# titoeb/RecModel

Hardware: AMD Instinct MI355X
Metric: ALS user+item row-updates/sec (higher is better)
Workload: dtype f32; 1 GPU; cfg3: WMF k=128+bias, 10000000x1000000 CSR, 99990947 nnz, alpha-log confidence, gamma=0.1, zipf_a=0.0; n_items=1000000, nnz=99990947, k=128, bias=True

## Files before the change

include/wmf_hip.h:

```cpp
#ifndef WMF_HIP_H
#define WMF_HIP_H

#include <stdint.h>

#ifdef __cplusplus
extern "C" {
#endif

#define WMF_OK            0
#define WMF_EINVAL       -1
#define WMF_EHIP         -2
#define WMF_ENOMEM       -3
#define WMF_ENUMERIC     -4

#define WMF_MAX_F        260

typedef struct wmf_plan wmf_plan;

const char* wmf_last_error(void);
int  wmf_version(void);
int  wmf_ld_for(int f);

int wmf_recompute_factors_host(const float* Y_host, int64_t m, int f, int bias,
                               const int64_t* indptr, const int32_t* indices, const float* values,
                               int64_t n, double lambda, float* X_host);

int64_t wmf_gram_workspace_bytes(int f);

int wmf_gram(const float* Y, int64_t m, int f, int ld, int bias,
             double* G_sum, void* workspace, void* stream);

int wmf_factorize(const double* G_sum, int f, int ld, double lambda,
                  float* W_white, float* W_unwhite, int32_t* info,
                  void* workspace, void* stream);

int wmf_rolled_layout_supported(int f, int ld);

int wmf_row_transform(const float* in, int64_t m, int f, int ld, const float* W,
                      int set_col0_one, float* out, float* col0_out, void* stream);
int wmf_whitened_row_floats(int f, int ld, int bias);

int wmf_chained_supported(int f, int ld, int bias);
int wmf_gram_whitened(const float* g, int64_t m, int f, int ld, int bias,
                      double* G_aug, void* workspace, void* stream);
int wmf_compose_whitening(const double* G_aug, const float* U, int f, int ld, int bias, int rolled, double lambda,
                          float* W_white, float* W_unwhite, float* N_ext, int32_t* info,
                          void* workspace, void* stream);
int wmf_row_transform_chained(const float* g, int64_t m, int f, int ld, int bias, const float* N_ext, int rolled,
                              float* out, float* col0_out, void* stream);

int  wmf_plan_create(const int64_t* indptr_host, int64_t n, int f, int bias, wmf_plan** out);
void wmf_plan_destroy(wmf_plan* p);
int  wmf_plan_stats(const wmf_plan* p, int64_t* out14);
int  wmf_plan_iter_stats(wmf_plan* p, int64_t* out4);

int wmf_solve_rows(const wmf_plan* plan, const float* V, const float* bias_fixed,
                   const int64_t* indptr, const int32_t* indices, const float* values,
                   int64_t n, int f, int ld, float* g, int32_t* fail_count, void* stream);
#define WMF_SOLVE_ROLLED 1
int wmf_solve_rows_ex(const wmf_plan* plan, const float* V, const float* bias_fixed,
                   const int64_t* indptr, const int32_t* indices, const float* values,
                   int64_t n, int f, int ld, float* g, int32_t* fail_count, int flags, void* stream);

int64_t wmf_eval_workspace_bytes(void);
int wmf_eval_sqerr(const float* users, const float* items, int f, int ld, int bias,
                   const int64_t* indptr, const int32_t* indices, const float* values,
                   int64_t n, double* out3, void* workspace, void* stream);

int64_t wmf_audit_workspace_bytes(int64_t n);
int wmf_half_step_audit(const float* X, const float* Y, int f, int ld, int bias,
                        const int64_t* indptr, const int32_t* indices, const float* values, int64_t n,
                        const double* dense, double* out_sums, double* out_rows,
                        void* workspace, int64_t workspace_bytes, void* stream);
int wmf_half_step_audit_f64(const double* X, const double* Y, int f, int bias,
                            const int64_t* indptr, const int32_t* indices, const double* values, int64_t n,
                            const double* dense, double* out_sums, double* out_rows,
                            void* workspace, int64_t workspace_bytes, void* stream);

#define WMF_EXPLAIN_MAX_TARGETS 16
int64_t wmf_explain_workspace_bytes(int64_t n, int f, int32_t n_targets);
int wmf_explain_rows(const float* Y, int64_t m, int f, int ld, int bias, const float* W_white,
                     const int64_t* indptr, const int32_t* indices, const float* values, int64_t n,
                     const int32_t* targets, int32_t n_targets,
                     float* out_contrib, float* out_total, int32_t* fail_count,
                     void* workspace, int64_t workspace_bytes, void* stream);

int64_t wmf_foldin_workspace_bytes(int64_t n, int f);
int wmf_foldin_rows(const float* Y, int64_t m, int f, int ld, int bias, const float* W_white,
                    const int64_t* indptr, const int32_t* indices, const float* values, int64_t n,
                    float* X_out, int32_t* fail_count,
                    void* workspace, int64_t workspace_bytes, void* stream);

int wmf_predict_pairs(const float* users, const float* items, int f, int ld, int bias,
                      const int32_t* users_idx, int64_t n_u, const int32_t* items_idx, int64_t n_i,
                      float* out, void* stream);

int64_t wmf_rank_workspace_bytes(int64_t n_cand);
// ... 178 lines not shown
```

recmodel_amd/_lib.py:

```python
import ctypes
import os

import torch

_HERE = os.path.dirname(os.path.abspath(__file__))
LIB_PATH = os.environ.get("WMF_HIP_LIB", os.path.join(_HERE, "libwmf_hip.so"))

WMF_OK, WMF_EINVAL, WMF_EHIP, WMF_ENOMEM, WMF_ENUMERIC = 0, -1, -2, -3, -4

c_int, c_i64, c_dbl, c_vp = ctypes.c_int, ctypes.c_int64, ctypes.c_double, ctypes.c_void_p

SIGNATURES = {
    "wmf_last_error": (ctypes.c_char_p, []),
    "wmf_version": (c_int, []),
    "wmf_ld_for": (c_int, [c_int]),
    "wmf_recompute_factors_host": (c_int, [c_vp, c_i64, c_int, c_int, c_vp, c_vp, c_vp, c_i64, c_dbl, c_vp]),
    "wmf_gram_workspace_bytes": (c_i64, [c_int]),
    "wmf_gram": (c_int, [c_vp, c_i64, c_int, c_int, c_int, c_vp, c_vp, c_vp]),
    "wmf_factorize": (c_int, [c_vp, c_int, c_int, c_dbl, c_vp, c_vp, c_vp, c_vp, c_vp]),
    "wmf_row_transform": (c_int, [c_vp, c_i64, c_int, c_int, c_vp, c_int, c_vp, c_vp, c_vp]),
    "wmf_whitened_row_floats": (c_int, [c_int, c_int, c_int]),
    "wmf_chained_supported": (c_int, [c_int, c_int, c_int]),
    "wmf_gram_whitened": (c_int, [c_vp, c_i64, c_int, c_int, c_int, c_vp, c_vp, c_vp]),
    "wmf_compose_whitening": (c_int, [c_vp, c_vp, c_int, c_int, c_int, c_int, c_dbl, c_vp, c_vp, c_vp, c_vp, c_vp, c_vp]),
# ... 42 lines not shown
                                 c_vp, c_vp, c_vp, c_vp, c_i64, c_vp]),
    "wmf_rerank_mmr_resident_pool": (c_i64, [c_int, c_int]),
    "wmf_rerank_mmr": (c_int, [c_vp, c_i64, c_int, c_int, c_int, c_vp, c_vp, c_vp, c_vp, c_i64, c_i64, ctypes.c_float, c_i64, c_vp, c_vp,
                               c_vp, c_vp, c_vp]),
    "wmf_intra_list_similarity": (c_int, [c_vp, c_i64, c_int, c_int, c_int, c_vp, c_vp, c_vp, c_i64, c_i64, c_vp, c_vp, c_vp]),
    "wmf_rank_positions_workspace_bytes": (c_i64, [c_i64, c_i64, c_int]),
    "wmf_rank_positions": (c_int, [c_vp, c_vp, c_int, c_int, c_int, c_vp, c_i64, c_i64, c_vp, c_vp, c_vp, c_vp, c_int, c_vp, c_vp,
                                   c_vp, c_i64, c_vp]),
    "wmf_hit_counts": (c_int, [c_vp, c_vp, c_int, c_int, c_int, c_vp, c_vp, c_vp, c_i64, c_vp, c_int, c_vp, c_vp, c_int, c_vp, c_vp]),
    "wmf_spmm_rows": (c_int, [c_vp, c_vp, c_vp, c_vp, c_i64, c_int, c_int, c_vp, c_vp]),
    "wmf_gather_rows": (c_int, [c_vp, c_int, c_vp, c_i64, c_vp, c_vp]),
    "wmf_coo_to_csr_workspace_bytes": (c_i64, [c_i64, c_i64, c_i64]),
    "wmf_coo_to_csr": (c_int, [c_vp, c_vp, c_vp, c_i64, c_i64, c_i64, c_vp, c_vp, c_vp, c_vp, c_vp, c_i64, c_vp]),
    "wmf_confidence_transform": (c_int, [c_vp, c_i64, c_dbl, c_dbl, c_int, c_vp]),
    "wmf_confidence_transform_f64": (c_int, [c_vp, c_i64, c_dbl, c_dbl, c_int, c_vp]),
    "wmf_half_step_f64_workspace_bytes": (c_i64, [c_int, c_i64, c_i64]),
    "wmf_half_step_f64": (c_int, [c_vp, c_i64, c_int, c_int, c_vp, c_vp, c_vp, c_i64, c_dbl, c_vp, c_vp, c_i64, c_vp, c_vp]),
    "wmf_recompute_factors_f64_host": (c_int, [c_vp, c_i64, c_int, c_int, c_vp, c_vp, c_vp, c_i64, c_dbl, c_vp]),
    "wmf_profile_enable": (c_int, [c_int]),
    "wmf_profile_set_tag": (c_int, [c_int]),
    "wmf_profile_collect": (c_int, []),
    "wmf_profile_entry": (c_int, [c_int, c_vp, c_int, c_vp, c_vp, c_vp, c_vp, c_vp]),
    "wmf_profile_reset": (c_int, []),
    "wmf_debug_set_flags": (c_int, [c_int]),
    "wmf_debug_get_flags": (c_int, []),
}

DEBUG_FLAGS = {
    "WMF_DBG_NO_ELIMINATION": 1,
    "WMF_DBG_NO_ACCUMULATION": 2,
    "WMF_DBG_NO_TILE_INVERSE": 8,
    "WMF_DBG_LOW32_GAUSS_JORDAN": 64,
    "WMF_DBG_NO_BORDER": 256,
    "WMF_DBG_WIDE_EIGHT_WAVES": 1024,
    "WMF_DBG_NO_ROW_PAIRS": 2048,
    "WMF_DBG_HEAVY_REG_RING": 4096,
    "WMF_DBG_HEAVY_F32_ACC": 8192,
    "WMF_DBG_HEAVY_REG_RING_K64": 65536,
    "WMF_DBG_F32_GRAM": 131072,
    "WMF_DBG_F32_TRANSFORM": 262144,
    "WMF_DBG_LOW_F32_TILES": 524288,
    "WMF_DBG_WIDE_F32": 2097152,
    "WMF_DBG_HEAVY_ONE_WAVE": 16777216,
    "WMF_DBG_HEAVY_PIVOTED_LU": 33554432,
    "WMF_DBG_F64_TEAMS": 67108864,
    "WMF_DBG_F64_NO_LOW_RANK": 134217728,
    "WMF_DBG_NO_ITER": 268435456,
    "WMF_DBG_F64_VALU": 536870912,
    "WMF_DBG_NO_ROLLED_LAYOUT": 1073741824,
}
SHIPPED_DEBUG_FLAGS = ("WMF_DBG_HEAVY_REG_RING", "WMF_DBG_F32_GRAM", "WMF_DBG_HEAVY_ONE_WAVE", "WMF_DBG_F64_NO_LOW_RANK",
                       "WMF_DBG_NO_ITER", "WMF_DBG_F64_VALU")


def parse_debug_flags(text):
    value = 0
    for part in str(text).split("|"):
        part = part.strip()
        name = part if part.startswith("WMF_DBG_") else "WMF_DBG_" + part
        value |= DEBUG_FLAGS[name] if name in DEBUG_FLAGS else int(part, 0)
    return value


class WmfLibraryError(RuntimeError):
    """libwmf_hip.so is missing or a HIP call failed."""


class WmfNumericError(ArithmeticError):
    """The Gramian was not positive definite or a row system was singular."""


_lib = None


def load():
    global _lib
    if _lib is not None:
        return _lib
    if not os.path.exists(LIB_PATH):
        raise WmfLibraryError(
            f"{LIB_PATH} is not built; run `python -c 'import __graft_entry__ as g; g.build()'` "
            "or `make -C recmodel_amd/csrc`.  There is no CPU fallback for the WMF hot path.")
    lib = ctypes.CDLL(LIB_PATH)
    for name, (res, args) in SIGNATURES.items():
        fn = getattr(lib, name)
        fn.restype, fn.argtypes = res, args
    flags = os.environ.get("WMF_DEBUG_FLAGS")
    if flags and lib.wmf_debug_set_flags(parse_debug_flags(flags)) != WMF_OK:
        raise ValueError(lib.wmf_last_error().decode("utf-8", "replace"))
    _lib = lib
    return lib


def profile_table(lib=None):
    lib = lib or load()
    out = []
    name = ctypes.create_string_buffer(200)
    tag, n = c_int(), c_i64()
    ms, lo, hi = c_dbl(), c_dbl(), c_dbl()
    for i in range(lib.wmf_profile_collect()):
        check(lib.wmf_profile_entry(i, name, 200, ctypes.byref(tag), ctypes.byref(ms), ctypes.byref(n), ctypes.byref(lo),
                                    ctypes.byref(hi)))
        out.append((name.value.decode(), tag.value, ms.value, n.value, lo.value, hi.value))
    return out


# ... 17 lines not shown
```

recmodel_amd/csrc/wmf_api.hip:

```cpp
#include "../../include/wmf_hip.h"
#include "wmf_internal.h"

#include <atomic>
#include <cstdarg>
#include <cstdio>
#include <cstring>
#include <mutex>
#include <set>
#include <string>
#include <vector>

static thread_local char g_err[512] = "";
int wmf_debug_flags = 0;

void wmf_set_error(const char* fmt, ...) {
    va_list ap;
    va_start(ap, fmt);
    vsnprintf(g_err, sizeof(g_err), fmt, ap);
    va_end(ap);
}

#define HIP_TRY(call)                                                                            \
    do {                                                                                         \
        hipError_t e_ = (call);                                                                  \
// ... 222 lines not shown
    double* gA = (double*)((char*)workspace + gram_a_off(f));
    wmf_launch_factorize(G_sum, f, ld, lambda, W_white, W_unwhite, info, gA, (hipStream_t)stream);
    return check_launch("wmf_factorize");
}

int wmf_row_transform(const float* in, int64_t m, int f, int ld, const float* W, int set_col0_one, float* out,
                      float* col0_out, void* stream) {
    int rc = check_shape(f, ld);
    if (rc) return rc;
    if (!in || !W || !out || m < 0) { wmf_set_error("wmf_row_transform: null pointer or negative m"); return WMF_EINVAL; }
    rc = wmf_launch_transform(in, m, f, ld, W, set_col0_one, out, col0_out, (hipStream_t)stream);
    if (rc) {
        if (rc == WMF_L_LAYOUT) wmf_set_error("wmf_row_transform: f=%d, ld=%d with set_col0_one writes the split layout: col0_out (float[2 m]) is required and out may not alias in", f, ld);
        else wmf_set_error("wmf_row_transform: unsupported f=%d", f);
        return WMF_EINVAL;
    }
    return check_launch("wmf_row_transform");
}

int wmf_chained_supported(int f, int ld, int bias) {
    if (check_shape(f, ld)) return 0;
    const int f1 = f + (bias ? 1 : 0);
    return (f >= 97 && f1 <= 144 && ld >= f1 && f + 1 <= WMF_MAX_F) ? 1 : 0;
}
static int check_chained(const char* what, int f, int ld, int bias) {
    if (wmf_chained_supported(f, ld, bias)) return WMF_OK;
    wmf_set_error("%s: unsupported f=%d, ld=%d, bias=%d (wmf_chained_supported)", what, f, ld, bias);
    return WMF_EINVAL;
}

int wmf_gram_whitened(const float* g, int64_t m, int f, int ld, int bias, double* G_aug, void* workspace, void* stream) {
    if (check_chained("wmf_gram_whitened", f, ld, bias)) return WMF_EINVAL;
    if (!g || !G_aug || !workspace || m < 0) { wmf_set_error("wmf_gram_whitened: null pointer or negative m"); return WMF_EINVAL; }
    {
        const int f1 = f + (bias ? 1 : 0);
        const int64_t nfb = (f1 + 15) / 16, nt = nfb * (nfb + 1) / 2;
        if ((int64_t)wmf_gram_nwaves(m, f1) * nt * 256 * (int64_t)sizeof(float) > gram_partial_bytes(f + 1)) {
            wmf_set_error("wmf_gram_whitened: workspace layout too small at f=%d", f);
            return WMF_EINVAL;
        }
    }
    if (wmf_launch_gram_aug(g, m, f, ld, bias, G_aug, (float*)workspace, (double*)((char*)workspace + gram_slices_off(f + 1)),
                            (hipStream_t)stream)) {
        wmf_set_error("wmf_gram_whitened: unsupported f=%d", f);
        return WMF_EINVAL;
    }
    return check_launch("wmf_gram_whitened");
}

int wmf_compose_whitening(const double* G_aug, const float* U, int f, int ld, int bias, int rolled, double lambda, float* W_white,
                          float* W_unwhite, float* N_ext, int32_t* info, void* workspace, void* stream) {
    if (check_chained("wmf_compose_whitening", f, ld, bias)) return WMF_EINVAL;
    if (!G_aug || !U || !W_white || !W_unwhite || !N_ext || !info || !workspace) { wmf_set_error("wmf_compose_whitening: null pointer"); return WMF_EINVAL; }
    if (rolled && !(bias && wmf_rolled_layout(f, ld))) { wmf_set_error("wmf_compose_whitening: rolled needs wmf_rolled_layout_supported(f=%d, ld=%d) and bias", f, ld); return WMF_EINVAL; }
    if (U == W_unwhite || U == W_white) { wmf_set_error("wmf_compose_whitening: U may not alias an output"); return WMF_EINVAL; }
    wmf_launch_compose(G_aug, U, f, ld, bias, rolled, lambda, W_white, W_unwhite, N_ext, info, (double*)workspace,
                       (double*)((char*)workspace + gram_a_off(f + 1)), (hipStream_t)stream);
    return check_launch("wmf_compose_whitening");
}

int wmf_row_transform_chained(const float* g, int64_t m, int f, int ld, int bias, const float* N_ext, int rolled, float* out,
                              float* col0_out, void* stream) {
    if (check_chained("wmf_row_transform_chained", f, ld, bias)) return WMF_EINVAL;
    if (!g || !N_ext || !out || m < 0) { wmf_set_error("wmf_row_transform_chained: null pointer or negative m"); return WMF_EINVAL; }
    const int rc = wmf_launch_transform_chained(g, m, f, ld, bias, N_ext, rolled, out, col0_out, (hipStream_t)stream);
    if (rc) {
        if (rc == WMF_L_LAYOUT) wmf_set_error("wmf_row_transform_chained: f=%d, ld=%d: col0_out is required with biases and out may not alias g in the split layout", f, ld);
        else wmf_set_error("wmf_row_transform_chained: unsupported f=%d, ld=%d, rolled=%d", f, ld, rolled);
        return WMF_EINVAL;
    }
    return check_launch("wmf_row_transform_chained");
}

static int bin_of(int64_t d, int f) {
    if (d <= 16) return WMF_BIN_LOW16;
    if (d <= 32) return WMF_BIN_LOW32;
    return wmf_direct_supported(f) ? WMF_BIN_MFMA : WMF_BIN_GENERAL;
}

int wmf_plan_create(const int64_t* indptr, int64_t n, int f, int bias, wmf_plan** out) {
    if (!indptr || !out || n < 0 || n > 0x7fffffffLL) { wmf_set_error("wmf_plan_create: bad arguments"); return WMF_EINVAL; }
    if (f < 1 || f > WMF_MAX_F) { wmf_set_error("wmf_plan_create: f=%d unsupported", f); return WMF_EINVAL; }
    wmf_plan* p = new wmf_plan();
    memset(p, 0, sizeof(*p));
    p->n = n; p->f = f;
    std::vector<int32_t> order((size_t)n);
    int64_t start[WMF_NBINS + 1] = {0};
    for (int64_t r = 0; r < n; ++r) {
        const int64_t d = indptr[r + 1] - indptr[r];
        if (d < 0) { delete p; wmf_set_error("wmf_plan_create: indptr not monotone at row %lld", (long long)r); return WMF_EINVAL; }
        p->count[bin_of(d, f)]++;
        p->nnz[bin_of(d, f)] += d;
    }
    for (int b = 0; b < WMF_NBINS; ++b) start[b + 1] = start[b] + p->count[b];
    int64_t fill[WMF_NBINS];
    for (int b = 0; b < WMF_NBINS; ++b) fill[b] = start[b];
    const int hb = wmf_direct_supported(f) ? WMF_BIN_MFMA : WMF_BIN_GENERAL;
    const bool can_split = wmf_direct_supported(f) || wmf_rowsplit_supported(f);
    std::vector<int32_t> heavy;
    for (int64_t r = 0; r < n; ++r) {
        const int64_t d = indptr[r + 1] - indptr[r];
        if (d <= 8) { order[(size_t)fill[WMF_BIN_LOW16]++] = (int32_t)r; p->count8++; p->nnz8 += d; }
    }
    const bool split_layout = bias && wmf_split_layout(f, wmf_ld_for(f));
    const int64_t iter_dmax = wmf_iter_dmax(f, wmf_ld_for(f), split_layout ? 1 : 0);
    p->iter_dmax = (int)iter_dmax;
    std::vector<int32_t> longer;
// ... 694 lines not shown
```

recmodel_amd/csrc/wmf_dense.hip:

```cpp
#include "wmf_common.h"
#include "wmf_internal.h"

#include <type_traits>
#include <utility>

template <int NFB, int NSPLIT, int S>
__device__ __forceinline__ void gram_body(const float* __restrict__ Y, int64_t m, int f, int ld, int bias,
                                          float* __restrict__ partial, int64_t step_lo, int64_t step_hi) {
    constexpr int NT = NFB * (NFB + 1) / 2;
    constexpr int NACC = (NT + NSPLIT - 1) / NSPLIT;
    const int lane = threadIdx.x & 63;
    const int r = lane & 15, q = lane >> 4;
    f32x4 acc[NACC];
#pragma unroll
    for (int i = 0; i < NACC; ++i) acc[i] = f32x4{0.f, 0.f, 0.f, 0.f};

    constexpr int U = 4;
    float cur[U][NFB], nxt[U][NFB];
    const int last_col = min(16 * (NFB - 1) + r, ld - 1);
    const float col_mask_last = (16 * (NFB - 1) + r < f) ? 1.f : 0.f;
    auto load_trip = [&](int64_t s0, float (&fr)[U][NFB]) {
#pragma unroll
        for (int uu = 0; uu < U; ++uu) {
            const int64_t row = min(4 * (s0 + uu) + q, m - 1);
// ... 342 lines not shown
        const int j = lane;
        double v = (i == j) ? 1.0 : 0.0;
        const double gv = G[min(i, f - 1) * f + min(j, f - 1)];
        if (i < f && j < f) v = gv + (i == j ? lambda : 0.0);
        Gs[i * FZ_LD + j] = v;
        Xs[i * FZ_LD + j] = 0.0;
    }
    __builtin_amdgcn_fence(__ATOMIC_RELEASE, "wavefront");
    __builtin_amdgcn_wave_barrier();
    int fail = 0;
    auto tile = [&](double* M, int bi, int bj) { return M + (16 * bi) * FZ_LD + 16 * bj; };
    auto sync = [&]() { __builtin_amdgcn_fence(__ATOMIC_RELEASE, "wavefront"); __builtin_amdgcn_wave_barrier(); };
    for (int p = 0; p < nb; ++p) {
        const int bad = fz_diag(tile(Gs, p, p), tile(Gs, p, p), tile(Xs, p, p), FZ_LD, lane);
        if (bad && !fail) fail = 16 * p + bad;
        sync();
        for (int i = p + 1; i < nb; ++i) {
            const f64x4 c = fz_mul_abt(tile(Gs, i, p), FZ_LD, tile(Xs, p, p), FZ_LD, f64x4{0.0, 0.0, 0.0, 0.0}, r, q, 1.0);
            sync();
            fz_store(tile(Gs, i, p), FZ_LD, c, r, q);
            sync();
        }
        for (int i = p + 1; i < nb; ++i)
            for (int j = p + 1; j <= i; ++j) {
                const f64x4 c = fz_mul_abt(tile(Gs, i, p), FZ_LD, tile(Gs, j, p), FZ_LD, fz_load(tile(Gs, i, j), FZ_LD, r, q), r, q, -1.0);
                fz_store(tile(Gs, i, j), FZ_LD, c, r, q);
            }
        sync();
    }
    for (int p = 0; p < nb; ++p)
        for (int i = p + 1; i < nb; ++i) {
            f64x4 sacc = f64x4{0.0, 0.0, 0.0, 0.0};
            for (int k = p; k < i; ++k) sacc = fz_mul_ab(tile(Gs, i, k), FZ_LD, tile(Xs, k, p), FZ_LD, sacc, r, q, 1.0);
            fz_store(Ts, FZ_LD, sacc, r, q);
            sync();
            const f64x4 c = fz_mul_ab(tile(Xs, i, i), FZ_LD, Ts, FZ_LD, f64x4{0.0, 0.0, 0.0, 0.0}, r, q, -1.0);
            fz_store(tile(Xs, i, p), FZ_LD, c, r, q);
            sync();
        }
    const bool ok = fail == 0;
    if (lane == 0 && !ok) *info = fail;
#pragma unroll 8
    for (int i = 0; i < 64; ++i) {
        if (i >= f) break;
        for (int j = lane; j < ld; j += 64) {
            float wu = 0.f, ww = 0.f;
            if (j < f && ok) { wu = (float)Xs[i * FZ_LD + j]; ww = (float)Xs[j * FZ_LD + i]; }
            Wunwhite[i * ld + j] = wu;
            Wwhite[i * ld + j] = ww;
        }
    }
}

__global__ __launch_bounds__(512, 1) void factorize_blocked_kernel(const double* __restrict__ G, int f, int ld, double lambda,
                                                                   float* __restrict__ Wwhite, float* __restrict__ Wunwhite,
                                                                   int32_t* __restrict__ info, double* __restrict__ work) {
    __shared__ __attribute__((aligned(16))) double Ts[8][16 * 18];
    __shared__ int bad;
    const int tid = threadIdx.x, lane = tid & 63, r = lane & 15, q = lane >> 4;
    const int wave = __builtin_amdgcn_readfirstlane(tid >> 6);
    const int nb = (f + 15) >> 4, fp = 16 * nb, LD = fp + 2;
    double* A = work;
    double* X = work + (size_t)fp * LD;
    if (tid == 0) bad = 0;
    for (int e = tid; e < fp * fp; e += 512) {
        const int i = e / fp, j = e % fp;
        double v = (i == j) ? 1.0 : 0.0;
        if (i < f && j < f) v = G[i * f + j] + (i == j ? lambda : 0.0);
        A[i * LD + j] = v;
        X[i * LD + j] = 0.0;
    }
    __syncthreads();
    auto tile = [&](double* M, int bi, int bj) { return M + (size_t)(16 * bi) * LD + 16 * bj; };
    for (int p = 0; p < nb; ++p) {
        if (wave == 0) {
            const int fail = fz_diag(tile(A, p, p), tile(A, p, p), tile(X, p, p), LD, lane);
            if (fail && lane == 0 && !bad) bad = 16 * p + fail;
        }
        __syncthreads();
        for (int i = p + 1 + wave; i < nb; i += 8) {
            const f64x4 c = fz_mul_abt(tile(A, i, p), LD, tile(X, p, p), LD, f64x4{0.0, 0.0, 0.0, 0.0}, r, q, 1.0);
            fz_store(tile(A, i, p), LD, c, r, q);
        }
        __syncthreads();
        int t = 0;
        for (int i = p + 1; i < nb; ++i)
            for (int j = p + 1; j <= i; ++j, ++t) {
                if ((t & 7) != wave) continue;
                const f64x4 c = fz_mul_abt(tile(A, i, p), LD, tile(A, j, p), LD, fz_load(tile(A, i, j), LD, r, q), r, q, -1.0);
                fz_store(tile(A, i, j), LD, c, r, q);
            }
        __syncthreads();
    }
    double* ts = Ts[wave];
    for (int p = wave; p < nb; p += 8)
        for (int i = p + 1; i < nb; ++i) {
            f64x4 sacc = f64x4{0.0, 0.0, 0.0, 0.0};
            for (int k = p; k < i; ++k) sacc = fz_mul_ab(tile(A, i, k), LD, tile(X, k, p), LD, sacc, r, q, 1.0);
            fz_store(ts, 18, sacc, r, q);
            __builtin_amdgcn_fence(__ATOMIC_RELEASE, "wavefront");
            __builtin_amdgcn_wave_barrier();
            const f64x4 c = fz_mul_ab(tile(X, i, i), LD, ts, 18, f64x4{0.0, 0.0, 0.0, 0.0}, r, q, -1.0);
            fz_store(tile(X, i, p), LD, c, r, q);
            __builtin_amdgcn_fence(__ATOMIC_RELEASE, "wavefront");
            __builtin_amdgcn_wave_barrier();
        }
    __syncthreads();
    const bool ok = bad == 0;
    if (tid == 0 && !ok) *info = bad;
    for (int e = tid; e < f * ld; e += 512) {
        const int i = e / ld, j = e % ld;
        float wu = 0.f, ww = 0.f;
        if (j < f && ok) { wu = (float)X[i * LD + j]; ww = (float)X[j * LD + i]; }
        Wunwhite[e] = wu;
        Wwhite[e] = ww;
    }
}

int wmf_launch_factorize(const double* G_sum, int f, int ld, double lambda, float* Wwhite, float* Wunwhite,
                         int32_t* info, double* gA, hipStream_t st) {
    if (f <= 64) {
        WmfProfScope ps("factorize64m_kernel", st);
        hipLaunchKernelGGL(factorize64m_kernel, dim3(1), dim3(64), 0, st, G_sum, f, ld, lambda, Wwhite, Wunwhite, info);
        return 0;
    }
    WmfProfScope ps("factorize_blocked_kernel", st);
    hipLaunchKernelGGL(factorize_blocked_kernel, dim3(1), dim3(512), 0, st, G_sum, f, ld, lambda, Wwhite, Wunwhite, info, gA);
    return 0;
}

template <int NFB, bool W_IN_LDS, int NB0 = 0, int NBW = NFB>
__global__ __launch_bounds__(512) void transform_kernel(const float* __restrict__ in, int64_t m, int f, int ld,
                                                        const float* __restrict__ W, int set_col0_one,
                                                        float* __restrict__ out, float* __restrict__ col0_out,
                                                        int64_t nblocks16) {
    extern __shared__ __attribute__((aligned(16))) char smem_raw[];
    float* Wl = reinterpret_cast<float*>(smem_raw);
    constexpr int KP = 16 * NFB;
    constexpr int NP = 16 * NBW;
    constexpr int LDW = NP + 4;
    const int tid = threadIdx.x;
    __shared__ int nz[NFB * NBW];
    for (int e = tid; e < NFB * NBW; e += 512) nz[e] = 0;
    __syncthreads();
    for (int e = tid; e < KP * LDW; e += 512) {
        const int a = e / LDW, b = e % LDW, col = 16 * NB0 + b;
        const float v = (a < f && b < NP && col < f) ? W[a * ld + col] : 0.f;
        if constexpr (W_IN_LDS) Wl[e] = v;
        if (v != 0.f) nz[(a >> 4) * NBW + (b >> 4)] = 1;
    }
    __syncthreads();
    const int lane = tid & 63, wv = tid >> 6;
    const int r = lane & 15, q = lane >> 4;
    const int nch = ld >> 2;
    unsigned tmask[NFB];
#pragma unroll
    for (int t = 0; t < NFB; ++t) {
        unsigned mk = 0;
#pragma unroll
        for (int nb = 0; nb < NBW; ++nb) mk |= nz[t * NBW + nb] ? (1u << nb) : 0u;
        tmask[t] = __builtin_amdgcn_readfirstlane(mk);
    }
    constexpr bool DBL = NFB <= 11;
    const int64_t stride = (int64_t)gridDim.x * 8;
    auto request = [&](int64_t blk, float4 (&x)[NFB]) {
        const int64_t row = blk * 16 + r;
        const float4* irow = reinterpret_cast<const float4*>(in + (row < m ? row : 0) * (int64_t)ld);
#pragma unroll
        for (int t = 0; t < NFB; ++t) x[t] = irow[min(4 * t + q, nch - 1)];
    };
    auto block = [&](int64_t blk, float4 (&xc)[NFB], float4 (&xn)[NFB]) {
        if constexpr (DBL) { if (blk + stride < nblocks16) request(blk + stride, xn); }
        const int64_t row = blk * 16 + r;
        const bool rok = row < m;
        f32x4 acc[NBW];
#pragma unroll
        for (int nb = 0; nb < NBW; ++nb) acc[nb] = f32x4{0.f, 0.f, 0.f, 0.f};
#pragma unroll
        for (int t = 0; t < NFB; ++t) {
            const int c = 4 * t + q;
// ... 263 lines not shown
            launch_transform_slice<NFB, H, NFB - H>(in, m, f, ld, W, set_col0_one, out, col0_out, grid, nblk, st);
        } else {
            launch_transform_slice<NFB, 0, 6>(in, m, f, ld, W, set_col0_one, out, col0_out, grid, nblk, st);
            launch_transform_slice<NFB, 6, 6>(in, m, f, ld, W, set_col0_one, out, col0_out, grid, nblk, st);
            launch_transform_slice<NFB, 12, NFB - 12>(in, m, f, ld, W, set_col0_one, out, col0_out, grid, nblk, st);
        }
    } else {
        static const char* nm = wmf_kname("transform_kernel<%d, false, 0, %d>", NFB, NFB);
        WMF_LAUNCH(nm, (transform_kernel<NFB, false>), dim3((unsigned)grid), dim3(512), 0, st, in, m, f, ld, W,
                   set_col0_one, out, col0_out, nblk);
    }
    return WMF_L_OK;
}

int wmf_launch_transform(const float* in, int64_t m, int f, int ld, const float* W, int set_col0_one, float* out,
                         float* col0_out, hipStream_t st) {
    if (m <= 0) return WMF_L_OK;
    const int nfb = (f + 15) / 16;
    if (set_col0_one == 3 || set_col0_one == 4) {
        if (!wmf_rolled_layout(f, ld)) return WMF_L_NO_KERNEL;
    } else {
        set_col0_one = set_col0_one ? (wmf_split_layout(f, ld) ? 2 : 1) : 0;
    }
    if ((set_col0_one == 2 || set_col0_one == 3) && (!col0_out || in == out)) return WMF_L_LAYOUT;
    return wmf_dispatch_nfb<1, 17>(nfb, [&](auto n) { return launch_transform_nfb<decltype(n)::value>(in, m, f, ld, W, set_col0_one, out, col0_out, st); });
}

__device__ __forceinline__ double compose_t(const float* __restrict__ U, int f, int ld, int bias, int rolled, int p, int j) {
    if (p >= f) return j == 0 ? 1.0 : 0.0;
    if (bias && j == 0) return 0.0;
    const int src = rolled ? (p + 1 == f ? 0 : p + 1) : p;
    return (double)U[src * ld + j];
}
template <class FA, class FB>
__device__ __forceinline__ double compose_dot16(int n, FA a, FB b) {
    double s = 0.0;
#pragma unroll 3
    for (int k = threadIdx.x & 15; k < n; k += 16) s += a(k) * b(k);
#pragma unroll
    for (int off = 8; off; off >>= 1) s += __shfl_xor(s, off, 16);
    return s;
}
__global__ __launch_bounds__(256) void compose_h_kernel(const double* __restrict__ Gaug, const float* __restrict__ U, int f, int ld,
                                                        int bias, int rolled, double* __restrict__ H) {
    const int f1 = f + (bias ? 1 : 0);
    const int e0 = (blockIdx.x * blockDim.x + threadIdx.x) >> 4;
    const bool live = e0 < f1 * f;
    const int e = live ? e0 : 0;
    const int p = e / f, j = e - p * f;
    const double s = compose_dot16(f1, [&](int k) { return Gaug[p * f1 + k]; }, [&](int k) { return compose_t(U, f, ld, bias, rolled, k, j); });
    if (live && (threadIdx.x & 15) == 0) H[e] = s;
}
__global__ __launch_bounds__(256) void compose_g_kernel(const double* __restrict__ H, const float* __restrict__ U, int f, int ld,
                                                        int bias, int rolled, double* __restrict__ Gt) {
    const int f1 = f + (bias ? 1 : 0);
    const int e0 = (blockIdx.x * blockDim.x + threadIdx.x) >> 4;
    const bool live = e0 < f * f;
    const int e = live ? e0 : 0;
    int i = e / f, j = e - i * f;
    if (i > j) { const int t = i; i = j; j = t; }
    const double s = compose_dot16(f1, [&](int p) { return compose_t(U, f, ld, bias, rolled, p, i); }, [&](int p) { return H[p * f + j]; });
    if (live && (threadIdx.x & 15) == 0) Gt[e] = s;
}
__global__ __launch_bounds__(256) void compose_n_kernel(const float* __restrict__ U, const float* __restrict__ Ww, int f, int ld,
                                                        int bias, int rolled, float* __restrict__ N) {
    const int f1 = f + (bias ? 1 : 0);
    const int e0 = (blockIdx.x * blockDim.x + threadIdx.x) >> 4;
    const bool live = e0 < f1 * ld;
    const int e = live ? e0 : 0;
    const int p = e / ld, n = e - p * ld;
    const int col = n >= f ? 0 : rolled ? (n + 1 == f ? 0 : n + 1) : n;
    double s = compose_dot16(f, [&](int j) { return compose_t(U, f, ld, bias, rolled, p, j); }, [&](int j) { return (double)Ww[j * ld + col]; });
    if (n >= f) s = (n == f && bias && p < f) ? (double)U[(rolled ? (p + 1 == f ? 0 : p + 1) : p) * ld] : 0.0;
    if (live && (threadIdx.x & 15) == 0) N[e] = (float)s;
}

int wmf_launch_compose(const double* G_aug, const float* U, int f, int ld, int bias, int rolled, double lambda, float* Wwhite,
                       float* Wunwhite, float* N_ext, int32_t* info, double* scratch, double* gA, hipStream_t st) {
    const int f1 = f + (bias ? 1 : 0);
    double* H = scratch;
    double* Gt = scratch + (size_t)f1 * f;
    WMF_LAUNCH("compose_h_kernel", compose_h_kernel, dim3((f1 * f + 15) / 16), dim3(256), 0, st, G_aug, U, f, ld, bias, rolled, H);
    WMF_LAUNCH("compose_g_kernel", compose_g_kernel, dim3((f * f + 15) / 16), dim3(256), 0, st, H, U, f, ld, bias, rolled, Gt);
    wmf_launch_factorize(Gt, f, ld, lambda, Wwhite, Wunwhite, info, gA, st);
    WMF_LAUNCH("compose_n_kernel", compose_n_kernel, dim3((f1 * ld + 15) / 16), dim3(256), 0, st, U, Wwhite, f, ld, bias, rolled, N_ext);
    return WMF_L_OK;
}

template <int NFB, int MODE>
__global__ __launch_bounds__(512) void chain6_kernel(const float* __restrict__ in, int64_t m, int f, int ld,
                                                     const float* __restrict__ W,
                                                     float* __restrict__ out, float* __restrict__ col0_out,
                                                     int64_t nblocks16) {
    extern __shared__ __attribute__((aligned(16))) char smem_raw[];
    constexpr int NP = 16 * NFB;
    constexpr int NKC = (NP + 31) / 32;
    constexpr int KS = 176;
    static_assert(32 * NKC <= KS, "K does not fit the LDS row");
    __bf16* Wt = reinterpret_cast<__bf16*>(smem_raw);
    __shared__ int nz[NKC * NFB];
    const int tid = threadIdx.x;
    constexpr bool bias = MODE != 0;
    const int f1 = f + (bias ? 1 : 0);
    for (int e = tid; e < NKC * NFB; e += 512) nz[e] = 0;
    __syncthreads();
    typedef __bf16 stage_bf16x8 __attribute__((ext_vector_type(8)));
    stage_bf16x8* Ws = reinterpret_cast<stage_bf16x8*>(Wt);
    for (int it = tid; it < NP * (KS / 8); it += 512) {
        const int k8 = it / NP, n = it - k8 * NP;
        float v[8];
#pragma unroll
        for (int j = 0; j < 8; ++j) {
            const int k = 8 * k8 + j;
            const bool in_w = k < f1 && n < f1;
            v[j] = W[in_w ? k * ld + n : 0];
            if (!in_w) v[j] = 0.f;
        }
        stage_bf16x8 ph, pm, pl;
        bool any = false;
#pragma unroll
        for (int j = 0; j < 8; ++j) {
            const __bf16 h = (__bf16)v[j];
            const float r1 = v[j] - (float)h;
            const __bf16 md = (__bf16)r1;
            ph[j] = h; pm[j] = md; pl[j] = (__bf16)(r1 - (float)md);
            any |= v[j] != 0.f;
        }
        const int at = (n * KS + 8 * k8) / 8;
        Ws[at] = ph;
        Ws[NP * KS / 8 + at] = pm;
        Ws[2 * NP * KS / 8 + at] = pl;
        if (any) nz[(k8 >> 2) * NFB + (n >> 4)] = 1;
    }
    __syncthreads();
    const int lane = tid & 63, wv = __builtin_amdgcn_readfirstlane(tid >> 6);
    const int r = lane & 15, q = lane >> 4;
    const int nch = ld >> 2;
    unsigned cmask[NKC];
#pragma unroll
    for (int c = 0; c < NKC; ++c) {
        unsigned mk = 0;
#pragma unroll
        for (int nb = 0; nb < NFB; ++nb) mk |= nz[c * NFB + nb] ? (1u << nb) : 0u;
        cmask[c] = __builtin_amdgcn_readfirstlane(mk);
    }
    typedef __bf16 bf16x8_t __attribute__((ext_vector_type(8)));
    const bf16x8_t* Wl = reinterpret_cast<const bf16x8_t*>(Wt);
    const int64_t stride = (int64_t)gridDim.x * 8;
    auto request = [&](int64_t blk, float4 (&x)[2 * NKC]) {
        const int64_t row = blk * 16 + r;
        const float4* irow = reinterpret_cast<const float4*>(in + (row < m ? row : 0) * (int64_t)ld);
#pragma unroll
        for (int c = 0; c < NKC; ++c) {
            x[2 * c] = irow[min(8 * c + 2 * q, nch - 1)];
            x[2 * c + 1] = irow[min(8 * c + 2 * q + 1, nch - 1)];
        }
    };
    constexpr bool sp = MODE == 2 || MODE == 3;
    const int fcol = f & 15;
    auto block = [&](int64_t blk, float4 (&xc)[2 * NKC]) {
        f32x4 acc[NFB];
#pragma unroll
        for (int nb = 0; nb < NFB; ++nb) acc[nb] = f32x4{0.f, 0.f, 0.f, 0.f};
#pragma unroll
        for (int c = 0; c < NKC; ++c) {
            const int k0 = 32 * c + 8 * q;
            float xe[8] = {xc[2 * c].x, xc[2 * c].y, xc[2 * c].z, xc[2 * c].w, xc[2 * c + 1].x, xc[2 * c + 1].y, xc[2 * c + 1].z, xc[2 * c + 1].w};
            if (32 * c + 32 > 16 * (NFB - 1)) {
#pragma unroll
                for (int e = 0; e < 8; ++e) if (!(k0 + e < f)) xe[e] = (bias && k0 + e == f) ? 1.f : 0.f;
            }
            bf16x8_t ah, am, al;
#pragma unroll
            for (int e = 0; e < 8; ++e) {
                const __bf16 h = (__bf16)xe[e];
                const float r1 = xe[e] - (float)h;
                const __bf16 md = (__bf16)r1;
                ah[e] = h; am[e] = md; al[e] = (__bf16)(r1 - (float)md);
            }
            unsigned mv = cmask[c];
            asm volatile("" : "+v"(mv));
            const unsigned mk = __builtin_amdgcn_readfirstlane(mv);
#pragma unroll
            for (int nb = 0; nb < NFB; ++nb) {
                if (!(mk & (1u << nb))) continue;
                const int at = ((16 * nb + r) * KS + 32 * c + 8 * q) / 8;
                const bf16x8_t bh = Wl[at], bm = Wl[NP * KS / 8 + at], bl = Wl[2 * NP * KS / 8 + at];
                f32x4 cc = acc[nb];
                cc = __builtin_amdgcn_mfma_f32_16x16x32_bf16(al, bh, cc, 0, 0, 0);
                cc = __builtin_amdgcn_mfma_f32_16x16x32_bf16(am, bm, cc, 0, 0, 0);
                cc = __builtin_amdgcn_mfma_f32_16x16x32_bf16(ah, bl, cc, 0, 0, 0);
                cc = __builtin_amdgcn_mfma_f32_16x16x32_bf16(am, bh, cc, 0, 0, 0);
                cc = __builtin_amdgcn_mfma_f32_16x16x32_bf16(ah, bm, cc, 0, 0, 0);
                cc = __builtin_amdgcn_mfma_f32_16x16x32_bf16(ah, bh, cc, 0, 0, 0);
                acc[nb] = cc;
            }
        }
        const int wid = sp ? f - 1 : ld;
        const bool stuff = MODE == 3 && (r & 7) < 2;
        const int stuff_sh = 2 * (r >> 3) + (r & 7);
        auto store_rows = [&](auto full) {
#pragma unroll
            for (int reg = 0; reg < 4; ++reg) {
                const int64_t orow = blk * 16 + 4 * q + reg;
                const float bias_src = acc[NFB - 1][reg];
                const unsigned bbits = MODE == 3 ? (unsigned)__builtin_amdgcn_ds_bpermute((16 * q + fcol) * 4, __builtin_bit_cast(int, bias_src)) : 0u;
                if (decltype(full)::value || orow < m) {
                    float* o = out + orow * (int64_t)wid;
#pragma unroll
                    for (int nb = 0; nb < NFB; ++nb) {
                        const int col = 16 * nb + r;
                        float v = acc[nb][reg];
                        if (MODE == 3 && 16 * nb < 128) {
                            const unsigned vb = __builtin_bit_cast(unsigned, v);
                            v = __builtin_bit_cast(float, stuff ? ((vb & ~1u) | ((bbits >> (4 * nb + stuff_sh)) & 1u)) : vb);
                        }
                        if (nb < NFB - 1) { o[col] = v; continue; }
                        if (col < wid) o[col] = col < f ? v : 0.f;
// ... 42 lines not shown
```

recmodel_amd/csrc/wmf_internal.h:

```cpp
#pragma once
#include <hip/hip_runtime.h>
#include <stdint.h>
#include <type_traits>
#include <utility>
#include "../../include/wmf_hip.h"
#include "wmf_filter.h"

#define WMF_GRAM_MAX_WAVES 4096
#define WMF_EVAL_MAX_BLOCKS 2048
#define WMF_AUDIT_MAX_BLOCKS 2048
#define WMF_HEAVY_T 4096
#define WMF_SEG 2048
#define WMF_WIDE_LU_GRID 64

extern int wmf_debug_flags;
#ifdef WMF_LAB
constexpr bool WMF_LAB_BUILD = true;
#else
constexpr bool WMF_LAB_BUILD = false;
#endif
constexpr int WMF_DBG_SHIPPED = WMF_DBG_HEAVY_REG_RING | WMF_DBG_F32_GRAM | WMF_DBG_HEAVY_ONE_WAVE | WMF_DBG_F64_NO_LOW_RANK |
                                WMF_DBG_NO_ITER | WMF_DBG_F64_VALU;
constexpr int WMF_DBG_LAB = WMF_DBG_NO_ELIMINATION | WMF_DBG_NO_ACCUMULATION | WMF_DBG_NO_TILE_INVERSE | WMF_DBG_LOW32_GAUSS_JORDAN |
                            WMF_DBG_NO_BORDER | WMF_DBG_WIDE_EIGHT_WAVES | WMF_DBG_NO_ROW_PAIRS | WMF_DBG_HEAVY_F32_ACC |
                            WMF_DBG_HEAVY_REG_RING_K64 | WMF_DBG_F32_TRANSFORM | WMF_DBG_LOW_F32_TILES | WMF_DBG_WIDE_F32 |
                            WMF_DBG_HEAVY_PIVOTED_LU | WMF_DBG_F64_TEAMS | WMF_DBG_NO_ROLLED_LAYOUT;
constexpr int WMF_DBG_ACCEPTED = WMF_LAB_BUILD ? (WMF_DBG_SHIPPED | WMF_DBG_LAB) : WMF_DBG_SHIPPED;

enum { WMF_BIN_LOW16 = 0, WMF_BIN_LOW32 = 1, WMF_BIN_MFMA = 2, WMF_BIN_GENERAL = 3, WMF_NBINS = 4 };

struct wmf_plan {
    int64_t n;
    int f;
    int64_t count[WMF_NBINS];
    int64_t count8, nnz8;
    bool bias;
    bool split;
    int64_t nnz[WMF_NBINS];
    int32_t* rows[WMF_NBINS];
    int32_t* rows_all;
    int32_t* fallback_rows;
    int32_t* fallback_count;
    float* w_eff;
    int64_t heavy_count, heavy_nnz, seg_total;
    int64_t* seg_lo;
    int32_t* seg_d;
    int32_t* seg_first;
    float* partial;
    float* wide_ws;
    int64_t iter_count, iter_nnz;
    int iter_dmax;
    int32_t* iter_bounce_rows;
    int32_t* iter_info;
    unsigned long long* iter_stats;
};

int wmf_gram_max_waves(int f);
int wmf_gram_nwaves(int64_t m, int f);
int wmf_launch_gram(const float* Y, int64_t m, int f, int ld, int bias, double* G_sum, float* partial, double* slices,
                    hipStream_t st);
int wmf_launch_factorize(const double* G_sum, int f, int ld, double lambda, float* Wwhite, float* Wunwhite,
                         int32_t* info, double* gA, hipStream_t st);
int wmf_launch_transform(const float* in, int64_t m, int f, int ld, const float* W, int set_col0_one, float* out,
                         float* col0_out, hipStream_t st);
int wmf_launch_gram_aug(const float* g, int64_t m, int f, int ld, int bias, double* G_aug, float* partial, double* slices,
                        hipStream_t st);
int wmf_launch_compose(const double* G_aug, const float* U, int f, int ld, int bias, int rolled, double lambda, float* Wwhite,
                       float* Wunwhite, float* N_ext, int32_t* info, double* scratch, double* gA, hipStream_t st);
int wmf_launch_transform_chained(const float* g, int64_t m, int f, int ld, int bias, const float* N_ext, int rolled, float* out,
                                 float* col0_out, hipStream_t st);

enum WmfLaunchRc { WMF_L_OK = 0, WMF_L_NO_KERNEL = -1, WMF_L_HIP = -2, WMF_L_LAYOUT = -3, WMF_L_TOO_MANY_KEYS = -4 };

struct RowArgs {
    const float* V; const float* side; const float* biasv; int bstride;
    const int64_t* indptr; const int32_t* indices; const float* vals;
    int f, ld; float* g; int32_t* fb_rows; int32_t* fb_count; int32_t* fail_count;
    int dbg; bool rolled; hipStream_t st;
};
struct RowList { const int32_t* rows; int64_t count; const int32_t* count_dev; };

template <int N>
using wmf_int = std::integral_constant<int, N>;
template <int... NS, class Fn>
static inline int wmf_dispatch_list(int n, Fn&& fn) {
    int rc = WMF_L_NO_KERNEL;
    (void)(... || (n == NS ? ((rc = fn(wmf_int<NS>{})), true) : false));
    return rc;
}
template <int LO, class Fn, int... IS>
static inline int wmf_dispatch_seq(int n, Fn&& fn, std::integer_sequence<int, IS...>) { return wmf_dispatch_list<(LO + IS)...>(n, fn); }
template <int LO, int HI, class Fn>
static inline int wmf_dispatch_nfb(int n, Fn&& fn) { return wmf_dispatch_seq<LO>(n, fn, std::make_integer_sequence<int, HI - LO + 1>{}); }
template <class Fn>
static inline int wmf_dispatch_dw(int f, bool border, Fn&& fn) {
    if (border) return wmf_dispatch_list<1, 2, 4, 5, 6, 8>(f / 16, [&](auto n) { return fn(n, std::true_type{}); });
    return wmf_dispatch_nfb<1, 9>((f + 15) / 16, [&](auto n) { return fn(n, std::false_type{}); });
}

int wmf_launch_solve(const wmf_plan* plan, const RowArgs& a);
static inline int wmf_direct_supported(int f) { return f >= 1 && f <= 144; }
static inline bool wmf_dw_border(int f) { return f > 16 && f <= 144 && f % 16 == 1 && (f / 16) % 4 != 3 && !(wmf_debug_flags & WMF_DBG_NO_BORDER); }
static inline bool wmf_split_layout(int f, int ld) { return wmf_dw_border(f) && ld == f + 3; }
int wmf_directl_supported(int f, int ld);
int wmf_launch_directl(const RowArgs& a, RowList l);
int wmf_launch_directl_segments(const wmf_plan* pl, const RowArgs& a);
int wmf_launch_directw(const wmf_plan* pl, const RowArgs& a);
int64_t wmf_directw_partial_floats(int f);
int wmf_launch_accumulate(const RowArgs& a, const int32_t* degrees, int64_t n, float* partial, int slot_stride, int slot_offset);
int wmf_launch_eliminate(const RowArgs& a, float* partial, int64_t n, int slots_per_row);
void wmf_launch_bias_adjust(const float* vals, const int32_t* indices, const float* biasv, int64_t nnz, float* w_eff,
                            hipStream_t st);
int64_t wmf_csr_ws_bytes(int64_t nnz, int64_t n_rows, int64_t n_cols);
int wmf_launch_coo_to_csr(const int64_t* rows, const int64_t* cols, const float* vals, int64_t nnz, int64_t n_rows, int64_t n_cols,
                          int64_t* indptr, int32_t* indices, float* values, int32_t* bad_flag, void* ws, hipStream_t st);
int wmf_wide_supported(int f);
int wmf_launch_wide(const RowArgs& a, RowList l);
int wmf_iter_dmax(int f, int ld, int split);
int wmf_launch_iter(const wmf_plan* pl, const RowArgs& a, RowList l);
static inline bool wmf_iter_enabled() { return !(wmf_debug_flags & WMF_DBG_NO_ITER); }
// ... 139 lines not shown
```

recmodel_amd/engine.py:

```python
import ctypes
import os

import numpy as np
import torch

from . import _lib


def _ptr(t):
    return ctypes.c_void_p(t.data_ptr()) if t is not None else None


def _stream():
    return ctypes.c_void_p(torch.cuda.current_stream().cuda_stream)


class _HeldWork:

    def __init__(self, work, *buffers, landing=None):
        self.work, self.buffers, self.landing = work, buffers, landing

    def wait(self):
        self.work.wait()
        if self.landing is not None:
# ... 707 lines not shown
    def _publish(self, side, c, force=False):
        if not self.exchange:
            return
        if self.reduce[self._other(side)] and not force:
            self._stale[side] = True
            return
        lo, ln = self.chunk_bounds[side][c]
        W = self.world
        if self.sparse[side]:
            need = self.need[side]
            start, stop = self.chunk_range[side][c]
            rows = need["send_idx"][c]
            send = self.K.gather_rows(self.factors[side], rows) if hasattr(self.K, "gather_rows") else self.factors[side].index_select(0, rows)
            self._pending[side].append(self._all_to_all_rows(self.X[side][start:stop], send, need["recv_counts"][c],
                                                             need["send_counts"][c]))
            return
        self._pending[side].append(torch.distributed.all_gather_into_tensor(
            self.X[side][W * lo: W * (lo + ln)], self.factors[side][lo: lo + ln], group=self.group, async_op=True))

    def _all_to_all_rows(self, out, send, recv_counts, send_counts):
        if torch.distributed.get_backend(self.group) == "nccl" or not out.is_cuda:
            work = torch.distributed.all_to_all_single(out, send, list(recv_counts), list(send_counts), group=self.group, async_op=True)
            return _HeldWork(work, send)
        torch.cuda.current_stream().synchronize()
        send_h, out_h = send.cpu(), torch.empty(out.shape, dtype=out.dtype)
        work = torch.distributed.all_to_all_single(out_h, send_h, list(recv_counts), list(send_counts), group=self.group, async_op=True)
        return _HeldWork(work, send_h, landing=(out, out_h))

    def _ensure_gathered(self, side):
        if self._stale[side]:
            self._stale[side] = False
            for c in range(len(self.chunk_bounds[side])):
                self._publish(side, c, force=True)
        self._wait(side)

    def _wait(self, side):
        for work in self._pending[side]:
            if work is not None:
                work.wait()
        self._pending[side] = []

    def _invalidate(self, side):
        self.g_valid[side] = self._owed[side] = False

    def _materialize(self, side):
        if self._owed[side]:
            self._owed[side] = False
            self.K.row_transform(self.g[side], self.n_local[side], self.f, self.ld, self.U[side], self.unwhite_mode,
                                 self.factors.raw(side), None)

    def _prepare_chained(self, fixed):
        K, n = self.K, self.n_local[fixed]
        K.gram_whitened(self.g[fixed], n, self.f, self.ld, self.bias, self.G_aug, self.ws)
        K.compose_whitening(self.G_aug, self.U[fixed], self.f, self.ld, self.bias, self.rolled, self.gamma, self.W_white,
                            self.W_unwhite, self.N_ext, self.info, self.ws)
        K.row_transform_chained(self.g[fixed], n, self.f, self.ld, self.bias, self.N_ext, self.rolled, self.V[fixed],
                                self.bias_vec[fixed] if self.bias else None)

    def prepare(self, fixed):
        K = self.K
        self._fixed_from_g = self.chained and self.g_valid[fixed]
        if self._fixed_from_g:
            return self._prepare_chained(fixed)
        blk = self.factors[fixed]
        K.gram(blk, self.n_local[fixed], self.f, self.ld, self.bias, self.G, self.ws)
        if self.exchange:
            torch.distributed.all_reduce(self.G, group=self.group)
        K.factorize(self.G, self.f, self.ld, self.gamma, self.W_white, self.W_unwhite, self.info, self.ws)
        V, bvec = self.V[fixed], self.bias_vec[fixed]
        if not self.exchange:
            K.row_transform(self.X[fixed], self.n_local[fixed], self.f, self.ld, self.W_white, self.white_mode, V,
                            bvec if self.bias else None)
            return
        if self._stale[fixed]:
            self._ensure_gathered(fixed)
        pending, self._pending[fixed] = self._pending[fixed], []
        done = len(self.chunk_bounds[fixed]) - len(pending)
        for c, (start, stop) in enumerate(self.chunk_range[fixed]):
            if c >= done and pending[c - done] is not None:
                pending[c - done].wait()
            rows = slice(start, stop)
            if stop > start:
                K.row_transform(self.X[fixed][rows], stop - start, self.f, self.ld, self.W_white, self.white_mode, V[rows],
                                bvec[rows] if self.bias else None)

    def update(self, side):
        K = self.K
        fixed = self._other(side)
        bvec = self.bias_vec[fixed] if self.bias else None
        self._wait(side)
        self._invalidate(side)
        for c, ((lo, ln), csr) in enumerate(zip(self.chunk_bounds[side], self.csr_chunks[side])):
            g = self.g[side][lo: lo + ln]
            K.solve_rows(csr._plan, self.V[fixed], bvec, csr.indptr, csr.indices, csr.values, ln, self.f, self.ld, g, self.fail,
                         self.solve_flags)
            if self.chained and self._fixed_from_g:
                continue
            real = max(0, min(ln, self.n_local[side] - lo))
            K.row_transform(g, real, self.f, self.ld, self.W_unwhite, self.unwhite_mode, self.factors.raw(side)[lo: lo + ln], None)
            self._publish(side, c)
        if self.chained:
            self.U[side].copy_(self.W_unwhite)
            self.g_valid[side] = True
            self._owed[side] = self._fixed_from_g
        self.has_factors[side] = True

    def half_step(self, side):
# ... 201 lines not shown
```

Before: 438.2 million row-updates/s.

## Reverse whitening permutation for users and special-case short K tail in chained transform

Adds a compose flag that reverses the index order of the composed Gramian before factorization when users are the fixed side. The whitening factor's triangular structure then lands in a different orientation, likely to keep the extra bias column out of a mostly empty K chunk. Separately, the chained row transform now handles a final K chunk of at most two live columns with scalar FMAs from a small LDS tail, skipping the MFMA pass for that chunk. The change adds plumbing for the permutation and carries risk around the correctness of the index mapping.

```diff
diff --git a/include/wmf_hip.h b/include/wmf_hip.h
--- a/include/wmf_hip.h
+++ b/include/wmf_hip.h
@@ -43,6 +43,8 @@
 int wmf_chained_supported(int f, int ld, int bias);
 int wmf_gram_whitened(const float* g, int64_t m, int f, int ld, int bias,
                       double* G_aug, void* workspace, void* stream);
+#define WMF_COMPOSE_ROLLED 1
+#define WMF_COMPOSE_REVERSED 2
 int wmf_compose_whitening(const double* G_aug, const float* U, int f, int ld, int bias, int rolled, double lambda,
                           float* W_white, float* W_unwhite, float* N_ext, int32_t* info,
                           void* workspace, void* stream);
diff --git a/recmodel_amd/_lib.py b/recmodel_amd/_lib.py
--- a/recmodel_amd/_lib.py
+++ b/recmodel_amd/_lib.py
@@ -118,6 +118,9 @@
 SHIPPED_DEBUG_FLAGS = ("WMF_DBG_HEAVY_REG_RING", "WMF_DBG_F32_GRAM", "WMF_DBG_HEAVY_ONE_WAVE", "WMF_DBG_F64_NO_LOW_RANK",
                        "WMF_DBG_NO_ITER", "WMF_DBG_F64_VALU")
 
+COMPOSE_ROLLED = 1
+COMPOSE_REVERSED = 2
+
 
 def parse_debug_flags(text):
     value = 0
diff --git a/recmodel_amd/csrc/wmf_api.hip b/recmodel_amd/csrc/wmf_api.hip
--- a/recmodel_amd/csrc/wmf_api.hip
+++ b/recmodel_amd/csrc/wmf_api.hip
@@ -298,7 +298,8 @@
                           float* W_unwhite, float* N_ext, int32_t* info, void* workspace, void* stream) {
     if (check_chained("wmf_compose_whitening", f, ld, bias)) return WMF_EINVAL;
     if (!G_aug || !U || !W_white || !W_unwhite || !N_ext || !info || !workspace) { wmf_set_error("wmf_compose_whitening: null pointer"); return WMF_EINVAL; }
-    if (rolled && !(bias && wmf_rolled_layout(f, ld))) { wmf_set_error("wmf_compose_whitening: rolled needs wmf_rolled_layout_supported(f=%d, ld=%d) and bias", f, ld); return WMF_EINVAL; }
+    if (rolled & ~(WMF_COMPOSE_ROLLED | WMF_COMPOSE_REVERSED)) { wmf_set_error("wmf_compose_whitening: unknown flag in rolled=%d", rolled); return WMF_EINVAL; }
+    if ((rolled & WMF_COMPOSE_ROLLED) && !(bias && wmf_rolled_layout(f, ld))) { wmf_set_error("wmf_compose_whitening: rolled needs wmf_rolled_layout_supported(f=%d, ld=%d) and bias", f, ld); return WMF_EINVAL; }
     if (U == W_unwhite || U == W_white) { wmf_set_error("wmf_compose_whitening: U may not alias an output"); return WMF_EINVAL; }
     wmf_launch_compose(G_aug, U, f, ld, bias, rolled, lambda, W_white, W_unwhite, N_ext, info, (double*)workspace,
                        (double*)((char*)workspace + gram_a_off(f + 1)), (hipStream_t)stream);
diff --git a/recmodel_amd/csrc/wmf_dense.hip b/recmodel_amd/csrc/wmf_dense.hip
--- a/recmodel_amd/csrc/wmf_dense.hip
+++ b/recmodel_amd/csrc/wmf_dense.hip
@@ -418,9 +418,13 @@
     }
 }
 
+__host__ __device__ __forceinline__ int wmf_perm(int j, int f, int perm) {
+    return perm == 0 ? j : perm == 1 ? (j == 0 ? 0 : f - j) : f - 1 - j;
+}
+
 __global__ __launch_bounds__(512, 1) void factorize_blocked_kernel(const double* __restrict__ G, int f, int ld, double lambda,
                                                                    float* __restrict__ Wwhite, float* __restrict__ Wunwhite,
-                                                                   int32_t* __restrict__ info, double* __restrict__ work) {
+                                                                   int32_t* __restrict__ info, double* __restrict__ work, int perm) {
     __shared__ __attribute__((aligned(16))) double Ts[8][16 * 18];
     __shared__ int bad;
     const int tid = threadIdx.x, lane = tid & 63, r = lane & 15, q = lane >> 4;
@@ -477,21 +481,21 @@
     for (int e = tid; e < f * ld; e += 512) {
         const int i = e / ld, j = e % ld;
         float wu = 0.f, ww = 0.f;
-        if (j < f && ok) { wu = (float)X[i * LD + j]; ww = (float)X[j * LD + i]; }
+        if (j < f && ok) { wu = (float)X[i * LD + wmf_perm(j, f, perm)]; ww = (float)X[j * LD + wmf_perm(i, f, perm)]; }
         Wunwhite[e] = wu;
         Wwhite[e] = ww;
     }
 }
 
 int wmf_launch_factorize(const double* G_sum, int f, int ld, double lambda, float* Wwhite, float* Wunwhite,
-                         int32_t* info, double* gA, hipStream_t st) {
+                         int32_t* info, double* gA, hipStream_t st, int perm) {
     if (f <= 64) {
         WmfProfScope ps("factorize64m_kernel", st);
         hipLaunchKernelGGL(factorize64m_kernel, dim3(1), dim3(64), 0, st, G_sum, f, ld, lambda, Wwhite, Wunwhite, info);
         return 0;
     }
     WmfProfScope ps("factorize_blocked_kernel", st);
-    hipLaunchKernelGGL(factorize_blocked_kernel, dim3(1), dim3(512), 0, st, G_sum, f, ld, lambda, Wwhite, Wunwhite, info, gA);
+    hipLaunchKernelGGL(factorize_blocked_kernel, dim3(1), dim3(512), 0, st, G_sum, f, ld, lambda, Wwhite, Wunwhite, info, gA, perm);
     return 0;
 }
 
@@ -861,12 +865,13 @@
     if (live && (threadIdx.x & 15) == 0) H[e] = s;
 }
 __global__ __launch_bounds__(256) void compose_g_kernel(const double* __restrict__ H, const float* __restrict__ U, int f, int ld,
-                                                        int bias, int rolled, double* __restrict__ Gt) {
+                                                        int bias, int rolled, double* __restrict__ Gt, int perm) {
     const int f1 = f + (bias ? 1 : 0);
     const int e0 = (blockIdx.x * blockDim.x + threadIdx.x) >> 4;
     const bool live = e0 < f * f;
     const int e = live ? e0 : 0;
     int i = e / f, j = e - i * f;
+    i = wmf_perm(i, f, perm); j = wmf_perm(j, f, perm);
     if (i > j) { const int t = i; i = j; j = t; }
     const double s = compose_dot16(f1, [&](int p) { return compose_t(U, f, ld, bias, rolled, p, i); }, [&](int p) { return H[p * f + j]; });
     if (live && (threadIdx.x & 15) == 0) Gt[e] = s;
@@ -884,14 +889,16 @@
     if (live && (threadIdx.x & 15) == 0) N[e] = (float)s;
 }
 
-int wmf_launch_compose(const double* G_aug, const float* U, int f, int ld, int bias, int rolled, double lambda, float* Wwhite,
+int wmf_launch_compose(const double* G_aug, const float* U, int f, int ld, int bias, int flags, double lambda, float* Wwhite,
                        float* Wunwhite, float* N_ext, int32_t* info, double* scratch, double* gA, hipStream_t st) {
     const int f1 = f + (bias ? 1 : 0);
+    const int rolled = (flags & WMF_COMPOSE_ROLLED) ? 1 : 0;
+    const int perm = !(flags & WMF_COMPOSE_REVERSED) ? 0 : bias ? 1 : 2;
     double* H = scratch;
     double* Gt = scratch + (size_t)f1 * f;
     WMF_LAUNCH("compose_h_kernel", compose_h_kernel, dim3((f1 * f + 15) / 16), dim3(256), 0, st, G_aug, U, f, ld, bias, rolled, H);
-    WMF_LAUNCH("compose_g_kernel", compose_g_kernel, dim3((f * f + 15) / 16), dim3(256), 0, st, H, U, f, ld, bias, rolled, Gt);
-    wmf_launch_factorize(Gt, f, ld, lambda, Wwhite, Wunwhite, info, gA, st);
+    WMF_LAUNCH("compose_g_kernel", compose_g_kernel, dim3((f * f + 15) / 16), dim3(256), 0, st, H, U, f, ld, bias, rolled, Gt, perm);
+    wmf_launch_factorize(Gt, f, ld, lambda, Wwhite, Wunwhite, info, gA, st, perm);
     WMF_LAUNCH("compose_n_kernel", compose_n_kernel, dim3((f1 * ld + 15) / 16), dim3(256), 0, st, U, Wwhite, f, ld, bias, rolled, N_ext);
     return WMF_L_OK;
 }
@@ -908,9 +915,18 @@
     static_assert(32 * NKC <= KS, "K does not fit the LDS row");
     __bf16* Wt = reinterpret_cast<__bf16*>(smem_raw);
     __shared__ int nz[NKC * NFB];
+    __shared__ float ntail[2][NP];
     const int tid = threadIdx.x;
     constexpr bool bias = MODE != 0;
     const int f1 = f + (bias ? 1 : 0);
+    constexpr int KB = 32 * (NKC - 1);
+    const bool short_tail = __builtin_amdgcn_readfirstlane(f1 - KB <= 2 ? 1 : 0) != 0;
+    for (int e = tid; e < 2 * NP; e += 512) {
+        const int k = KB + e / NP, n = e % NP;
+        const bool in_w = k < f1 && n < f1;
+        const float v = W[in_w ? k * ld + n : 0];
+        ntail[e / NP][n] = in_w ? v : 0.f;
+    }
     for (int e = tid; e < NKC * NFB; e += 512) nz[e] = 0;
     __syncthreads();
     typedef __bf16 stage_bf16x8 __attribute__((ext_vector_type(8)));
@@ -969,10 +985,29 @@
     const int fcol = f & 15;
     auto block = [&](int64_t blk, float4 (&xc)[2 * NKC]) {
         f32x4 acc[NFB];
-#pragma unroll
-        for (int nb = 0; nb < NFB; ++nb) acc[nb] = f32x4{0.f, 0.f, 0.f, 0.f};
+        if (short_tail) {
+            const float4 xt = xc[2 * (NKC - 1)];
+            const float v0 = KB < f ? xt.x : (bias && KB == f) ? 1.f : 0.f;
+            const float v1 = KB + 1 < f ? xt.y : (bias && KB + 1 == f) ? 1.f : 0.f;
+            float a0[4], a1[4];
+#pragma unroll
+            for (int reg = 0; reg < 4; ++reg) {
+                a0[reg] = __builtin_bit_cast(float, __builtin_amdgcn_ds_bpermute((4 * q + reg) * 4, __builtin_bit_cast(int, v0)));
+                a1[reg] = __builtin_bit_cast(float, __builtin_amdgcn_ds_bpermute((4 * q + reg) * 4, __builtin_bit_cast(int, v1)));
+            }
+#pragma unroll
+            for (int nb = 0; nb < NFB; ++nb) {
+                const float n0 = ntail[0][16 * nb + r], n1 = ntail[1][16 * nb + r];
+                acc[nb] = f32x4{__builtin_fmaf(a0[0], n0, a1[0] * n1), __builtin_fmaf(a0[1], n0, a1[1] * n1),
+                                __builtin_fmaf(a0[2], n0, a1[2] * n1), __builtin_fmaf(a0[3], n0, a1[3] * n1)};
+            }
+        } else {
+#pragma unroll
+            for (int nb = 0; nb < NFB; ++nb) acc[nb] = f32x4{0.f, 0.f, 0.f, 0.f};
+        }
 #pragma unroll
         for (int c = 0; c < NKC; ++c) {
+            if (c == NKC - 1 && short_tail) break;
             const int k0 = 32 * c + 8 * q;
             float xe[8] = {xc[2 * c].x, xc[2 * c].y, xc[2 * c].z, xc[2 * c].w, xc[2 * c + 1].x, xc[2 * c + 1].y, xc[2 * c + 1].z, xc[2 * c + 1].w};
             if (32 * c + 32 > 16 * (NFB - 1)) {
diff --git a/recmodel_amd/csrc/wmf_internal.h b/recmodel_amd/csrc/wmf_internal.h
--- a/recmodel_amd/csrc/wmf_internal.h
+++ b/recmodel_amd/csrc/wmf_internal.h
@@ -60,12 +60,12 @@
 int wmf_launch_gram(const float* Y, int64_t m, int f, int ld, int bias, double* G_sum, float* partial, double* slices,
                     hipStream_t st);
 int wmf_launch_factorize(const double* G_sum, int f, int ld, double lambda, float* Wwhite, float* Wunwhite,
-                         int32_t* info, double* gA, hipStream_t st);
+                         int32_t* info, double* gA, hipStream_t st, int perm = 0);
 int wmf_launch_transform(const float* in, int64_t m, int f, int ld, const float* W, int set_col0_one, float* out,
                          float* col0_out, hipStream_t st);
 int wmf_launch_gram_aug(const float* g, int64_t m, int f, int ld, int bias, double* G_aug, float* partial, double* slices,
                         hipStream_t st);
-int wmf_launch_compose(const double* G_aug, const float* U, int f, int ld, int bias, int rolled, double lambda, float* Wwhite,
+int wmf_launch_compose(const double* G_aug, const float* U, int f, int ld, int bias, int flags, double lambda, float* Wwhite,
                        float* Wunwhite, float* N_ext, int32_t* info, double* scratch, double* gA, hipStream_t st);
 int wmf_launch_transform_chained(const float* g, int64_t m, int f, int ld, int bias, const float* N_ext, int rolled, float* out,
                                  float* col0_out, hipStream_t st);
diff --git a/recmodel_amd/engine.py b/recmodel_amd/engine.py
--- a/recmodel_amd/engine.py
+++ b/recmodel_amd/engine.py
@@ -783,7 +783,8 @@
     def _prepare_chained(self, fixed):
         K, n = self.K, self.n_local[fixed]
         K.gram_whitened(self.g[fixed], n, self.f, self.ld, self.bias, self.G_aug, self.ws)
-        K.compose_whitening(self.G_aug, self.U[fixed], self.f, self.ld, self.bias, self.rolled, self.gamma, self.W_white,
+        flags = (_lib.COMPOSE_ROLLED if self.rolled else 0) | (_lib.COMPOSE_REVERSED if fixed == "users" else 0)
+        K.compose_whitening(self.G_aug, self.U[fixed], self.f, self.ld, self.bias, flags, self.gamma, self.W_white,
                             self.W_unwhite, self.N_ext, self.info, self.ws)
         K.row_transform_chained(self.g[fixed], n, self.f, self.ld, self.bias, self.N_ext, self.rolled, self.V[fixed],
                                 self.bias_vec[fixed] if self.bias else None)
```

Result: faster. 446.3 million row-updates/s (median of 6 runs) (+1.9%).
